# cs2mosa/Heterogeneous-MOE-for-Diffusion-models

Measured on AMD Instinct MI355X. Metric: denoise-steps/sec (fwd+bwd) on 4x32x32 latents, higher is better.
Workload: dtype bf16

## Files before the change

heterogeneous-moe-for-diffusion-models_amd/csrc/bwd6.hip:

```cpp
#include "common.h"
#include "conv_args.h"
#include "conv6_common.h"
#include "hdmoe.h"
#include "conv6_body.h"
#include "conv7_body.h"
#include "wgrad6_body.h"
#include "wgrad7_body.h"
#include "wgrad8_body.h"
#include "conv6s_body.h"

namespace {

template <int MT, int NT, int TWS, int OT>
__global__ __launch_bounds__(512) void bwd6_kernel(C6Args c, W6Args a3, W6Args a5, int G6, int ibs, int obs) {
  const int b = blockIdx.x;
  if (b < G6) { conv6_body<MT, NT>(c, b, G6); return; }
  int r = b - G6;
  const int bx = r % ibs; r /= ibs;
  const int by = r % obs;
  const int z = r / obs;
  if (z < a3.chunks) wgrad6_body<3, TWS, OT, false>(a3, bx, by, z);
  else wgrad6_body<5, TWS, OT, false>(a5, bx, by, z - a3.chunks);
}

// ... 21 lines not shown
      else if (pairs == 2) wgrad8_body3<2, 8>(a3, bx, by, z);
      else wgrad8_body3<2, 16>(a3, bx, by, z);
      return;
    }
    r -= n3;
    const int bx = r % ibs; r /= ibs;
    wgrad7_body<5>(a5, bx, r % obs, r / obs);
  } else if (OT > 0) {
    const int bx = r % ibs; r /= ibs;
    const int by = r % obs;
    const int z = r / obs;
    if (z < a3.chunks) wgrad6_body<3, TWS, OT == 0 ? 1 : OT, false>(a3, bx, by, z);
    else wgrad6_body<5, TWS, OT == 0 ? 1 : OT, false>(a5, bx, by, z - a3.chunks);
  }
}

template <int CO, int KMASK, int TWS, int OT, int EPI = 0, bool DBG = false>
void launch_bwd7(const C7Plan& cp, const W6DualPlan& wp, hipStream_t stream) {
  if constexpr (!DBG && EPI == 0 && (TWS == 5 || OT == 2)) {
    if (cp.a.stamps || cp.a.dbg) { launch_bwd7<CO, KMASK, TWS, OT, 0, true>(cp, wp, stream); return; }
  }
  static unsigned long long attr = 0;
  if (hdmoe_first_on_device(attr)) { (void)hipFuncSetAttribute((const void*)bwd7_kernel<CO, KMASK, TWS, OT, EPI, DBG>, hipFuncAttributeMaxDynamicSharedMemorySize, 160 * 1024); }
  const size_t clds = cp.lds + (EPI ? C7Lds<TWS == 4>::film_extra(CO) : 0);
  const size_t lds = clds > wp.lds ? clds : wp.lds;
  const int obs = OT == 0 ? wp.c[0].Cout / 32 : wp.obs;
  unsigned nw = (unsigned)(wp.ibs * obs * (wp.c[0].chunks + wp.c[1].chunks));
  if (OT == 0) nw = (unsigned)((wp.c[0].Cin / (32 * wp.c[0].icw)) * (wp.c[0].Cout / (32 * wp.c[0].ocw)) * wp.c[0].chunks + wp.ibs * obs * wp.c[1].chunks);
  hipLaunchKernelGGL((bwd7_kernel<CO, KMASK, TWS, OT, EPI, DBG>), dim3(cp.G + nw), dim3(512), lds, stream, cp.a, wp.c[0], wp.c[1], (int)cp.G, wp.ibs, obs);
}

template <int NT, int TWS, int OT>
__global__ __launch_bounds__(512) void bwd6s_kernel(C6SArgs c, W6Args a3, int G6, int ibs, int obs) {
  const int b = blockIdx.x;
  if (b < G6) { conv6s_body<NT>(c, b, G6); return; }
  int r = b - G6;
  const int bx = r % ibs; r /= ibs;
  wgrad6_body<3, TWS, OT, true>(a3, bx, r % obs, r / obs);
}
template <int NT, int TWS, int OT>
void launch_bwd6s(const C6SPlan& cp, const W6DualPlan& wp, hipStream_t stream) {
  static unsigned long long attr = 0;
  if (hdmoe_first_on_device(attr)) { (void)hipFuncSetAttribute((const void*)bwd6s_kernel<NT, TWS, OT>, hipFuncAttributeMaxDynamicSharedMemorySize, 160 * 1024); }
  const size_t lds = cp.lds > wp.lds ? cp.lds : wp.lds;
  const unsigned grid = cp.G + (unsigned)(wp.ibs * wp.obs * wp.c[0].chunks);
  hipLaunchKernelGGL((bwd6s_kernel<NT, TWS, OT>), dim3(grid), dim3(512), lds, stream, cp.sa, wp.c[0], (int)cp.G, wp.ibs, wp.obs);
}
// ... 72 lines not shown
  C7Plan cp7;
  if (conv7_plan(c, dtype, cp7) || cp7.kmask != 3 || (cp7.w16 != 0) != (wp.TWS == 4)) return 1;
  const bool big = wp.TWS == 5, small = wp.TWS == 4 && cp7.CO == 2 && wp.OT == 2;
  if (!big && !small) return 1;
  cp7.a.film_u = film_u; cp7.a.film_e = film_e; cp7.a.film_mask = film_mask; cp7.a.film_de = film_de;
  cp7.a.film_inv = film_p > 0.f ? 1.f / (1.f - film_p) : 1.f;
  hdmoe_count_selection(HDMOE_SEL_FILM_DGRAD);
  if (big) {
    hdmoe_count_selection(HDMOE_SEL_BWD7_32);
    if (wp.c[0].chunks) {
      hdmoe_count_selection(HDMOE_SEL_BWD7_32_WGRAD8);
      hdmoe_count_selection(wp.c[0].icw == 2 ? (wp.c[0].ocw == 2 ? HDMOE_SEL_WGRAD8_C22 : HDMOE_SEL_WGRAD8_C21)
                                             : (wp.c[0].ocw == 2 ? HDMOE_SEL_WGRAD8_C12 : HDMOE_SEL_WGRAD8_C11));
    }
    if (wp.c[1].chunks) hdmoe_count_selection(HDMOE_SEL_BWD7_32_WGRAD7);
    if (cp7.CO == 2) launch_bwd7<2, 3, 5, 0, 1>(cp7, wp, stream); else launch_bwd7<1, 3, 5, 0, 1>(cp7, wp, stream);
  } else {
    hdmoe_count_selection(HDMOE_SEL_BWD7_16_OT2);
    launch_bwd7<2, 3, 4, 2, 1>(cp7, wp, stream);
  }
  return hdmoe_launch_status();
}

}
```

heterogeneous-moe-for-diffusion-models_amd/csrc/conv7.hip:

```cpp
#include "conv_args.h"
#include "hdmoe.h"
#include "conv7_body.h"

namespace {

template <int CO, int KMASK, bool W16, bool DBG>
__global__ __launch_bounds__(512) void conv7_kernel(C7Args a) { conv7_body<CO, KMASK, W16, 0, DBG>(a, blockIdx.x, gridDim.x); }

}

constexpr int C7_MIN_IMAGES = 192;
extern "C" int hdmoe_conv7_min_images(void) { return C7_MIN_IMAGES; }

int conv7_plan(const ConvArgs& c, int dtype, C7Plan& plan) {
  if (dtype != HDMOE_BF16 || c.stride != 1 || c.ones || c.Cphys != c.Cin || c.Ipad != c.Cin || c.Cin % 32 || c.Cin > 256 || c.Cstore != c.Cout) return 1;
  if (c.Cout % 32 || c.Cout > 256) return 1;
  const bool w16 = c.H == 16;
  if (!((c.H == 32 && c.W == 32) || (c.H == 16 && c.W == 16)) || c.Ho != c.H || c.Wo != c.W || c.N < C7_MIN_IMAGES) return 1;
  int kmask = 0;
  long maxtaps = 0;
  for (int g = 0; g < c.ngroups; ++g) {
    const int k = c.kh[g];
    if (c.kw[g] != k || (k != 3 && k != 5 && k != 7) || c.pt[g] != (k - 1) / 2 || c.pl[g] != (k - 1) / 2) return 1;
    kmask |= k == 3 ? 1 : (k == 5 ? 2 : 4);
    if ((long)k * k > maxtaps) maxtaps = (long)k * k;
  }
  const long xbytes = (long)c.N * c.H * c.W * c.Cin * 2;
  const long wbytes = ((long)(c.ngroups - 1) * c.wstride + maxtaps * c.Cout * c.Cin) * 2;
  if (!conv_align_extent_ok({c.x, c.w, c.y, c.res}, {xbytes, wbytes, (long)c.N * c.H * c.W * c.Cout})) return 1;
  const long gstride = c.wstride * 2, tapstride = (long)c.Cout * c.Cin * 2, imgstride = (long)c.H * c.W * c.Cin * 2;
  if ((gstride & 7) || (c.ngroups - 1) * gstride + maxtaps * tapstride >= (1l << 31) || c.N * imgstride >= (1l << 31)) return 1;
  C7Args& a = plan.a;
  a.x = c.x; a.w = c.w; a.y = c.y; a.res = c.res; a.seg = c.seg;
  a.N = c.N; a.Cin = c.Cin; a.Cout = c.Cout; a.ngroups = c.ngroups; a.alpha = c.alpha; a.beta = c.beta;
  a.xbytes = (int)xbytes; a.wbytes = (int)wbytes;
  a.dbg = 0;
  a.film_u = nullptr; a.film_e = nullptr; a.film_mask = nullptr; a.film_de = nullptr; a.film_inv = 1.f;
  a.stamps = (unsigned long long*)hdmoe_debug_stamp_buffer();
  conv_sort_groups_desc(c.kh, a.order, c.ngroups);
  for (int i = 0; i < HDMOE_MAX_GROUPS; ++i) a.gk[i] = (int)(a.order[i] * gstride) | c.kh[a.order[i]];
  const long gcap = 256;
  const long units = w16 ? (c.N + 1) / 2 + c.ngroups : c.N;
  plan.G = (unsigned)(units < gcap ? units : gcap);
  plan.CO = c.Cout % 64 == 0 ? 2 : 1;
  a.tapstride = (int)tapstride; a.blkstride = 32 * plan.CO * c.Cin * 2;
  a.imgstride = (int)imgstride; a.rowstride = c.W * c.Cin * 2;
  plan.w16 = w16 ? 1 : 0;
  plan.lds = w16 ? C7Lds<true>::BYTES : C7Lds<false>::BYTES;
  plan.kmask = (kmask & 4) ? 7 : 3;
  return 0;
}

template <int CO, int KMASK, bool W16, bool DBG>
static void conv7_launch_t(const C7Plan& p, hipStream_t stream) {
  static unsigned long long attr = 0;
  if (hdmoe_first_on_device(attr)) { (void)hipFuncSetAttribute((const void*)conv7_kernel<CO, KMASK, W16, DBG>, hipFuncAttributeMaxDynamicSharedMemorySize, C7Lds<W16>::BYTES); }
  hipLaunchKernelGGL((conv7_kernel<CO, KMASK, W16, DBG>), dim3(p.G), dim3(512), C7Lds<W16>::BYTES, stream, p.a);
}

void conv7_launch(const C7Plan& p, hipStream_t stream) {
// ... 17 lines not shown
```

heterogeneous-moe-for-diffusion-models_amd/csrc/conv7_body.h:

```cpp
#pragma once
#include <type_traits>
#include <utility>
#include "common.h"
#include "conv6_common.h"

namespace {

struct C7Args {
  const void* x; const void* w; void* y; const void* res; const int* seg;
  int N, Cin, Cout, ngroups;
  int order[HDMOE_MAX_GROUPS];
  int gk[HDMOE_MAX_GROUPS];
  int tapstride, blkstride;
  int imgstride, rowstride;
  float alpha, beta;
  int xbytes, wbytes;
  int dbg;
  unsigned long long* stamps;
  const void* film_u;
  const float* film_e;
  const unsigned char* film_mask;
  float* film_de;
  float film_inv;
};

template <bool W16> struct C7Geo;
template <> struct C7Geo<false> {
  static constexpr int IMG = 32, MB = 4, ROWB = 35 * 64, TILE = (32 * 35 + 3) * 64, WBUF = 8192, TCO = 4, PPW = 8, HBOFF = 0;
  static constexpr int ZBYTES = 38 * 64;
};
template <> struct C7Geo<true> {
  static constexpr int IMG = 16, MB = 2, ROWB = 19 * 64, TILE = (32 * 19 + 3) * 64, WBUF = 28672, TCO = 14, PPW = 4, HBOFF = 16 * 19 * 64;
  static constexpr int ZBYTES = HBOFF + 22 * 64;
};
template <bool W16> struct C7Lds {
  using GEO = C7Geo<W16>;
  static constexpr int T0 = 2 * GEO::WBUF;
  static constexpr int ZROW = T0 + 2 * GEO::TILE;
  static constexpr int TAB = ZROW + GEO::ZBYTES;
  static constexpr int BYTES = TAB + HDMOE_MAX_GROUPS * 16;
  static constexpr int film_bytes(int co) { return 8 * (W16 ? 2 : 1) * 32 * co * 4; }
  static constexpr bool film_in_ring(int co) { return BYTES + film_bytes(co) > 160 * 1024; }
  static constexpr int film_extra(int co) { return film_in_ring(co) ? 0 : film_bytes(co); }
};

template <int KS, int CO, int TCO> struct C7Sched {
// ... 281 lines not shown
              *reinterpret_cast<bf16x8*>(Y + o) = out;
            }
          }
#pragma unroll
          for (int j = 0; j < 8; ++j) {
#pragma unroll
            for (int off = 1; off < (W16 ? 16 : 32); off <<= 1) ds[j] += __shfl_xor(ds[j], off);
          }
          if ((r & (W16 ? 15 : 31)) == 0) {
            float* dst = part + (wave * NIMG + (W16 ? (r >> 4) : 0)) * NCH + 32 * b + 16 * p + 8 * h;
            *reinterpret_cast<float4*>(dst) = make_float4(ds[0], ds[1], ds[2], ds[3]);
            *reinterpret_cast<float4*>(dst + 4) = make_float4(ds[4], ds[5], ds[6], ds[7]);
          }
        }
      asm volatile("s_waitcnt lgkmcnt(0)\n\ts_barrier" ::: "memory");
      if (tid < NIMG * NCH) {
        const int img = tid / NCH, c = tid % NCH;
        const int n = img ? cur.n2 : cur.n;
        float sum = 0.f;
#pragma unroll
        for (int w = 0; w < 8; ++w) sum += part[(w * NIMG + img) * NCH + c];
        if (n >= 0) a.film_de[(long)n * a.Cout + cobase + c] = sum;
      }
    } else if (!(dbg & 4)) {
      bf16* Y = (bf16*)a.y;
      const bf16* R = (const bf16*)a.res;
      const int nimg = W16 ? ((r >> 4) ? cur.n2 : cur.n) : cur.n;
      const bool live = !W16 || nimg >= 0;
#pragma unroll
      for (int m = 0; m < MB; ++m) {
        const long pix = W16 ? (((long)nimg * 16 + 2 * wave + m) * 16 + (r & 15)) * a.Cout
                             : (((long)nimg * 32 + 4 * wave + m) * 32 + r) * a.Cout;
#pragma unroll
        for (int b = 0; b < CO; ++b)
#pragma unroll
          for (int p = 0; p < 2; ++p) {
            float v[8];
#pragma unroll
            for (int e = 0; e < 8; ++e) v[e] = a.alpha * acc[m][b][8 * p + e];
            if (R && live) {
              const long o0 = pix + cobase + 32 * b + 16 * p + 4 * h;
              const bf16x4 r0 = *reinterpret_cast<const bf16x4*>(R + o0);
              const bf16x4 r1 = *reinterpret_cast<const bf16x4*>(R + o0 + 8);
#pragma unroll
              for (int e = 0; e < 4; ++e) { v[e] += a.beta * (float)r0[e]; v[4 + e] += a.beta * (float)r1[e]; }
            }
// ... 37 lines not shown
```

heterogeneous-moe-for-diffusion-models_amd/hdmoe_hip/ops.py:

```python
from __future__ import annotations

import ctypes
import functools
import math
from typing import Optional, Sequence, Tuple, Union

import torch

from . import bank as _bank
from ._lib import dtype_code_cast
from ._lib import BF16, _int_array, call, dtype_code, lib

Tensor = torch.Tensor

F32S = 2
ROUTE_CONV6S = 6


def _c(t: Optional[Tensor]) -> Optional[Tensor]:
    if t is None:
        return None
    return t if t.is_contiguous() else t.contiguous()


# ... 373 lines not shown
        if w6:
            return lambda: _conv_record(x, seg, N, Ho * Wo, O, I, khs, kws, "split_bf16" if split else None, wgrad_name=w6)
        return lambda: _conv_record(x, seg, N, Ho * Wo, O, I, khs, kws, wgrad_name=_kernel_label(_route(
            "hdmoe_conv_wgrad_route", 34, N, H, W, Ho, Wo, I, Cphys, O, 1, ones, G, seg is not None, khs, kws, pts, pts, _dt(x),
            x.data_ptr() % 16 == 0 and dy.data_ptr() % 16 == 0), x, wgrad=True))
    w6 = "wgrad6_kernel<split>" if split else "wgrad6_kernel"
    if (x.dtype == torch.bfloat16 or split) and not ones and Ho == H and Wo == W and Cphys == I:
        dtc = F32S if split else _dt(x)
        kib = _w6_kib(G, N, H, W, I, O, khs, kws, dtc)
        ws = _w6_workspace("arena", x.device, kib) if bank is not None and _prof_ok() else None
        if ws is not None:
            if _timed("conv_wgrad", rec(w6 + " (deferred reduce)"), "hdmoe_conv_wgrad6", x, dy, Gs, seg, G, N, H, W, I, O, khs, kws, pts, pts, ws, ws.numel() * 4,
                      dtc, 1) == 0:
                bank.defer_w6(Gs, seg, ws, G, N, H, W, I, O, dtc, khs)
                STATS["w6_defer"] += 1
                return
        ws = _w6_workspace("stream", x.device, kib)
        if ws is not None:
            if _timed("conv_wgrad", rec(w6 + " (+ reduce)"), "hdmoe_conv_wgrad6", x, dy, Gs, seg, G, N, H, W, I, O, khs, kws, pts, pts, ws, ws.numel() * 4, dtc, 0) == 0:
                return
    _timed("conv_wgrad", rec(), "hdmoe_conv_wgrad", x, dy, Gs, seg, G, N, H, W, Ho, Wo, I, Cphys, O, 1, 1 if ones else 0, khs, kws, pts, pts, _dt(x))


_ConvCall = _collections.namedtuple("_ConvCall", "G gain_val alpha beta ones training normalize split res_raw out film")


class _MPConvFn(torch.autograd.Function):

    @staticmethod
    def forward(ctx, x, res, seg, c: _ConvCall, *tensors):
        G, gain_val, alpha, beta, ones, training, normalize, split = c.G, c.gain_val, c.alpha, c.beta, c.ones, c.training, c.normalize, c.split
        weights, gains = tensors[:G], list(tensors[G:]) or None
        ctx.film = getattr(x, "_film_rec", None) if FILM_DGRAD and x.is_contiguous() else None
        if ctx.film is not None:
            ctx.film.register()
        x = _c(x)
        N, H, W, Cphys = x.shape
        O, I = int(weights[0].shape[0]), int(weights[0].shape[1])
        khs = [_kernel_hw(w)[0] for w in weights]
        kws = [_kernel_hw(w)[1] for w in weights]
        pts = [(kw - 1) // 2 for kw in kws]
        Hos = {H + (kw - 1) - kh + 1 for kh, kw in zip(khs, kws)}
        if len(Hos) != 1:
            raise ValueError("grouped conv: all groups must produce the same output size")
        if any(w.shape[0] != O or w.shape[1] != I for w in weights):
            raise ValueError("grouped conv: all groups must share (out_channels, in_channels)")
        if I != Cphys + (1 if ones else 0):
            raise RuntimeError(f"MP_Conv: input has {Cphys} channels, weight expects {I}")
        Ho, Wo = Hos.pop(), W
        Ipad = (I + 15) // 16 * 16
        Opad = (O + 15) // 16 * 16
        taps = max(a * b for a, b in zip(khs, kws))
        wstride, wdstride = taps * O * Ipad, taps * I * Opad
        wdt, planes, dtc = (torch.bfloat16, 2, F32S) if split else (x.dtype, 1, _dt(x))
        L = ctx.layer = _ConvLayer(G, N, H, W, Ho, Wo, Cphys, I, O, Ipad, Opad, khs, kws, pts, wstride, wdstride, dtc, gain_val, alpha, beta, ones,
                               normalize, split, c.res_raw, res is not None)
        ent = None
        if _bank.ACTIVE is not None and gains is None:
# ... 29 lines not shown
                    seg, G, wstride, N, H, W, Ho, Wo, I, Cphys, Ipad, O, O, 1, 1 if ones else 0, khs, kws, pts, pts, dtc)
            _timed("conv_fwd", lambda: _fwd_record(*args), "hdmoe_conv_fwd", *args)
        ctx.save_for_backward(x, seg, *tensors)
        return y

    @staticmethod
    def backward(ctx, dy):
        x, seg, *tensors = ctx.saved_tensors
        L, nig = ctx.layer, ctx.needs_input_grad
        weights, gains = tensors[:L.G], list(tensors[L.G:]) or None
        dy = _c(dy)
        need_gain = gains is not None and any(nig[4 + L.G:])
        need_w = any(nig[4:4 + L.G]) or need_gain
        fused, dx = _conv_fused_bwd(ctx, L, x, dy, seg, nig[0]) if need_w and ctx.ent is not None else (False, None)
        if nig[0] and not fused:
            dx = _conv_dgrad(L, x, dy, ctx.wd, seg)
        dres = None
        if L.has_res and nig[1]:
            if L.res_raw or L.beta == 1.0:
                dres = dy
            else:
                dres = torch.empty_like(dy)
                call("hdmoe_axpby", dres, dy, None, L.beta, 0.0, dy.numel(), _dt(dy))
        dws, dgs = _conv_wgrad(ctx, L, x, dy, seg, weights, gains, need_gain) if need_w and not fused else ([None] * L.G, [None] * len(gains or ()))
        return (dx, dres, None, None, *dws, *dgs)


def _conv_fused_bwd(ctx, L: _ConvLayer, x, dy, seg, need_dx: bool):
    rec = ctx.film
    if rec is not None:
        rec.clear()
    plan = _conv_bwd_plan(L, seg, need_dx, ctx.ones6, x.device)
    ws = plan.workspace(L, x.device) if plan is not None and plan.policy is not None else None
    if plan is None or (ws is None and plan.policy is not None):
        return False, None
    if callable(plan.mid):
        plan = plan._replace(mid=plan.mid())
    dx = torch.empty_like(x) if need_dx else None
    fused = False
    if plan.film and rec is not None and FILM_DGRAD and need_dx and rec.sole_consumer(x):
        de = torch.empty(rec.e.shape, dtype=torch.float32, device=x.device)
        fused = plan._replace(name="hdmoe_conv_bwd6_film", tail=(rec.u, rec.e, rec.mask, de, rec.p, plan.dtc),
                              label=lambda: dict(plan.label(), name="bwd7_kernel (FiLM epilogue)")).launch(ctx.bank, ctx.ent, x, dy, dx, ws)
        if fused:
            rec.offer(dx, de)
            STATS["film_dgrad"] += 1
    fused = fused or plan.launch(ctx.bank, ctx.ent, x, dy, dx, ws)
    return fused, dx if fused else None


def _conv_dgrad(L: _ConvLayer, x, dy, wd, seg) -> Tensor:
    dx = torch.empty_like(x)
    pt_d = [kh - 1 - p for kh, p in zip(L.khs, L.pts)]
    pl_d = [kw - 1 - p for kw, p in zip(L.kws, L.pts)]
    args = (dy, wd, dx, None, L.alpha, 0.0,
            seg, L.G, L.wdstride, L.N, L.Ho, L.Wo, L.H, L.W, L.O, L.O, L.Opad, L.I, L.Cphys, 1, 0, L.khs, L.kws, pt_d, pl_d, L.dtc)
    _timed("conv_fwd", lambda: _fwd_record(*args), "hdmoe_conv_fwd", *args)
    return dx


def _conv_wgrad(ctx, L: _ConvLayer, x, dy, seg, weights, gains, need_gain: bool):
    G, O, I = L.G, L.O, L.I
    geom = (seg, G, L.N, L.H, L.W, L.Ho, L.Wo, I, L.Cphys, O, L.ones, L.khs, L.kws, L.pts, L.split)
    dgs = [None] * len(gains or ())
    if ctx.ent is not None:
        _wgrad(x, dy, ctx.ent.G, *geom, bank=ctx.bank)
        ctx.bank.note_backward(ctx.ent)
        return [None] * G, dgs
    sizes = [kh * kw * O * I for kh, kw in zip(L.khs, L.kws)]
# ... 73 lines not shown
def _mp_conv(x, weights, gain=1.0, *, seg=None, res=None, alpha=1.0, beta=0.0, ones=False, training=False, normalize=True, split=False,
             res_grad_raw=False, out: Optional[Tensor] = None, film: Optional["_FilmReq"] = None) -> Tensor:
    ws = f32_params(list(weights) if isinstance(weights, (list, tuple)) else [weights])
    G = len(ws)
    if isinstance(gain, (list, tuple)):
        gts, gain_val = f32_params(list(gain)), 1.0
    elif torch.is_tensor(gain):
        gts, gain_val = f32_params([gain]) * G, 1.0
    else:
        gts, gain_val = [], float(gain)
    shape = x.shape
    grouped = seg is not None
    if x.ndim not in (2, 3, 4):
        raise ValueError("mp_conv: x must be 2-, 3- or 4-D")
    pointwise = all(w.ndim == 2 or (w.shape[2] == 1 and w.shape[3] == 1) for w in ws)
    if pointwise and not grouped and not ones:
        x4 = x.reshape(1, 1, -1, shape[-1])
    elif x.ndim == 2:
        x4 = x.reshape(shape[0], 1, 1, shape[1])
    elif x.ndim == 3:
        x4 = x.reshape(shape[0], 1, shape[1], shape[2])
    else:
        x4 = x
    if res is not None:
        res = res.reshape(x4.shape[0], x4.shape[1], x4.shape[2], -1)
    split = bool(split) and not ones and x4.dtype == torch.float32 and _split_ok(*x4.shape, ws)
    c = _ConvCall(G, gain_val, float(alpha), float(beta), bool(ones), bool(training), bool(normalize), split, bool(res_grad_raw), out, film)
    y = _MPConvFn.apply(x4, res, seg, c, *ws, *gts)
    return y.reshape(*shape[:-1], y.shape[-1])


class _MultiLinearFn(torch.autograd.Function):

    @staticmethod
    def forward(ctx, x, seg, ents, bank, c, *tensors):
        x = _f32(x)
        R, I = x.shape
        L = len(ents)
        G = len(ents[0].params)
        Os = [e.O for e in ents]
        ys = [torch.empty((R, o), dtype=torch.float32, device=x.device) for o in Os]
        call("hdmoe_mlinear_fwd", ys, x, [e.wf for e in ents], seg, Os, L, R, I, ents[0].Ipad, G, c)
        ctx.save_for_backward(x, seg)
        ctx.meta = (ents, bank, Os, G)
        return tuple(ys)

    @staticmethod
    def backward(ctx, *gs):
        x, seg = ctx.saved_tensors
        ents, bank, Os, G = ctx.meta
# ... 438 lines not shown
    def backward(ctx, g):
        return _FilmSiluFn.backward(ctx, g) + (None,)


def mp_conv_film(x: Tensor, weights, gain, emb: Tensor, p: float, training: bool, seg: Optional[Tensor] = None) -> Tensor:
    p = float(p) if training else 0.0
    C = int((weights[0] if isinstance(weights, (list, tuple)) else weights).shape[0])
    ok = (CONV_FILM and (p == 0.0 or CONV_FILM_TRAIN) and x.dtype == torch.bfloat16 and x.ndim == 4 and C % 8 == 0 and 256 % (C // 8) == 0
          and _bank.ACTIVE is not None)
    if not ok:
        return film_silu(mp_conv(x, weights, gain, seg=seg, training=training), emb, p, training)
    req = _FilmReq(_f32(emb), p, _next_seed() if p > 0.0 else 0)
    y = _mp_conv(x, weights, gain, seg=seg, training=training, film=req)
    if req.h is not None:
        return _FilmDoneFn.apply(y, req.emb, p, req.seed, req.h)
    return _FilmSiluFn.apply(y, req.emb, p, req.seed)


ONES6 = True
BLK6 = True
BLK6_SCOPE = "c32"


def unet_block_fused(h: Tensor, res: Optional[Tensor], w1s, w2s, gain1: float, gain2: float, emb: Tensor, p: float, training: bool,
                     seg: Optional[Tensor], alpha: float, beta: float, res_grad_raw: bool = False) -> Optional[Tensor]:
    w1s, w2s = list(w1s), list(w2s)
    if not (BLK6 and _bank.ACTIVE is not None and _prof_ok() and h.dtype == torch.bfloat16 and h.ndim == 4 and h.is_cuda):
        return None
    if res is not None and (res.dtype != h.dtype or not res.is_contiguous()):
        return None
    ent1 = _bank.ACTIVE.lookup(w1s, h.dtype, float(gain1), 1.0, True)
    ent2 = _bank.ACTIVE.lookup(w2s, h.dtype, float(gain2), float(alpha), True)
    if ent1 is None or ent2 is None or ent1.khs != ent1.kws or ent1.khs != ent2.khs or ent2.khs != ent2.kws:
        return None
    h = _c(h)
    N, H, W, Cin = h.shape
    C = ent1.O
    if ent1.I != Cin or ent2.I != C or ent2.O != C or (seg is None and len(w1s) != 1):
        return None
    if BLK6_SCOPE == "c32" and (C != 32 or (H == 32 and W == 32 and N >= _c7_min_images())):
        return None
    p = float(p) if training else 0.0
    e32 = _f32(emb)
    seed = _next_seed() if p > 0.0 else 0
    y = torch.empty((N, H, W, C), dtype=h.dtype, device=h.device)
    need_bwd = torch.is_grad_enabled() and (h.requires_grad or emb.requires_grad or any(w.requires_grad for w in w1s + w2s))
    u = torch.empty_like(y) if need_bwd else None
    hb = torch.empty_like(y) if need_bwd else None
    if _timed("fused", dict(name="blk6_kernel (fwd)", dtype="bfloat16", seg=seg, N=N, HW=H * W, O=C, I=Cin + C, taps=[k * k for k in ent1.khs], mult=1.0),
              "hdmoe_unet_block_fwd", h, ent1.wf, ent2.wf, u, hb, y, res, e32, seed, step_counter(h.device), p, float(alpha), float(beta), seg,
              len(w1s), ent1.wstride, ent2.wstride, N, H, W, Cin, C, ent1.khs, _dt(h)) != 0:
        if p > 0.0:
            _seed_state["ctr"] -= 1
        return None
    STATS["blk"] += 1
    if not need_bwd:
        return y
    ws1 = w1s if seg is not None else w1s[0]
    ws2 = w2s if seg is not None else w2s[0]
    uu = _mp_conv(h, ws1, gain1, seg=seg, training=training, out=u)
    hh = _FilmDoneFn.apply(uu, e32, p, seed, hb)
    return _mp_conv(hh, ws2, gain2, seg=seg, res=res, alpha=alpha, beta=beta, training=training, res_grad_raw=res_grad_raw, out=y)

# ... 42 lines not shown
        Ca, Cb = a.shape[-1], b.shape[-1]
        rows = a.numel() // Ca
        out = torch.empty((*a.shape[:-1], Ca + Cb), dtype=a.dtype, device=a.device)
        call("hdmoe_cat2_fwd", out, a, b, wa, wb, Ca, Cb, rows, _dt(a))
        ctx.meta = (wa, wb, a.shape, b.shape)
        return out

    @staticmethod
    def backward(ctx, g):
        wa, wb, sa, sb = ctx.meta
        g = _c(g)
        da = torch.empty(sa, dtype=g.dtype, device=g.device)
        db = torch.empty(sb, dtype=g.dtype, device=g.device)
        call("hdmoe_cat2_bwd", da, db, g, wa, wb, sa[-1], sb[-1], da.numel() // sa[-1], _dt(g))
        return da, db, None, None


def mp_cat(a: Tensor, b: Tensor, t: float = 0.5) -> Tensor:
    na, nb = a.shape[-1], b.shape[-1]
    c = math.sqrt((na + nb) / ((1.0 - t) ** 2 + t ** 2))
    return _Cat2Fn.apply(a, b, c * (1.0 - t) / math.sqrt(na), c * t / math.sqrt(nb))


class _SiluBranchFn(torch.autograd.Function):

    @staticmethod
    def forward(ctx, x, gx_scale):
        ctx.set_materialize_grads(False)
        x = _c(x)
        h = torch.empty_like(x)
        call("hdmoe_mp_silu_fwd", h, x, x.numel(), _dt(x))
        ctx.save_for_backward(x)
        ctx.sx = float(gx_scale)
        return x.view(x.shape), h

    @staticmethod
    def backward(ctx, gx, gh):
        (x,) = ctx.saved_tensors
        if gh is None:
            if gx is None or ctx.sx == 1.0:
                return gx, None
            dx = torch.empty_like(x)
            call("hdmoe_axpby", dx, _c(gx), None, ctx.sx, 0.0, dx.numel(), _dt(dx))
            return dx, None
        gh = _c(gh)
        dx = torch.empty_like(x)
        if gx is None:
            call("hdmoe_mp_silu_bwd", dx, gh, x, x.numel(), _dt(x))
        else:
            call("hdmoe_mp_silu_bwd_add", dx, gh, x, _c(gx), ctx.sx, x.numel(), _dt(x))
        return dx, None


class _CatSiluFn(torch.autograd.Function):

    @staticmethod
    def forward(ctx, a, b, wa, wb):
        ctx.set_materialize_grads(False)
        a = _c(a); b = _c(b)
        Ca, Cb = a.shape[-1], b.shape[-1]
        out = torch.empty((*a.shape[:-1], Ca + Cb), dtype=a.dtype, device=a.device)
        h = torch.empty_like(out)
        call("hdmoe_cat2_silu_fwd", out, h, a, b, wa, wb, Ca, Cb, a.numel() // Ca, _dt(a))
        ctx.save_for_backward(out)
        ctx.meta = (wa, wb, a.shape, b.shape)
        return out, h

    @staticmethod
    def backward(ctx, gcat, gh):
        (out,) = ctx.saved_tensors
        wa, wb, sa, sb = ctx.meta
        da = torch.empty(sa, dtype=out.dtype, device=out.device)
        db = torch.empty(sb, dtype=out.dtype, device=out.device)
        if gh is None:
            if gcat is None:
                return None, None, None, None
            call("hdmoe_cat2_bwd", da, db, _c(gcat), wa, wb, sa[-1], sb[-1], da.numel() // sa[-1], _dt(out))
        else:
            call("hdmoe_cat2_silu_bwd", da, db, None if gcat is None else _c(gcat), _c(gh), out, wa, wb, sa[-1], sb[-1], da.numel() // sa[-1], _dt(out))
        return da, db, None, None


def _vec_ok(*ts) -> bool:
    return all(t.shape[-1] % (8 if t.dtype == torch.bfloat16 else 4) == 0 and t.dtype in (torch.bfloat16, torch.float32) for t in ts)


def silu_branch(x: Tensor, gx_scale: float = 1.0):
    if _vec_ok(x) and x.numel() % 8 == 0:
        return _SiluBranchFn.apply(x, float(gx_scale))
    x, xh = fanout(x, 2)
    if gx_scale != 1.0:
        x = affine_grad(x, gx_scale)
    return x, mp_silu(xh)

# ... 1587 lines not shown
```

heterogeneous-moe-for-diffusion-models_amd/models/model_components.py:

```python
from __future__ import annotations

from typing import List, Optional, Sequence

import torch
import torch.nn as nn

import models.model_internals as m
from hdmoe_hip import ops

Tensor = torch.Tensor


class Scaling_router(nn.Module):

    def __init__(self, emb_dim: Optional[int] = 3, num_experts: Optional[int] = 2, dropout: Optional[float] = 0.2):
        super().__init__()
        self.soft_route = nn.Sequential(
            m.MP_Conv(in_channels=emb_dim, out_channels=emb_dim * 2, kernel=()),
            nn.GroupNorm(1, emb_dim * 2),
            nn.ReLU(),
            m.MP_Conv(in_channels=emb_dim * 2, out_channels=emb_dim * 4, kernel=()),
            nn.GroupNorm(1, emb_dim * 4),
            nn.ReLU(),
            nn.Dropout(dropout),
# ... 92 lines not shown

    def conv(name, inp, gain=1.0, **kw):
        return ops.mp_conv(inp, [getattr(b, name).weights for b in blocks], gain, seg=seg, training=tr, **kw)

    emb = film if film is not None else ops.affine(conv("emb_layer", embedding, b0.emb_gain), 1.0, 1.0)
    x = ops.resample(x, b0.resample)
    t = b0.residual_balance
    n = ((1.0 - t) ** 2 + t ** 2) ** 0.5
    beta = (1.0 - t) / n
    raw = False
    if b0.type == "enc":
        if b0.conv_skip is not None:
            x = conv("conv_skip", x)
        x, h = ops.pixel_norm_silu(x, gx_scale=beta)
        raw = True
    elif silu_x is not None:
        h = silu_x
    else:
        skip_next = b0.conv_skip is not None
        x, h = ops.silu_branch(x, gx_scale=1.0 if skip_next else beta)
        raw = not skip_next
    w1, w2 = [b.conv_res1.weights for b in blocks], [b.conv_res2.weights for b in blocks]
    if b0.type == "dec" and b0.conv_skip is not None:
        x = conv("conv_skip", x, alpha=beta)
        rbeta, raw = 1.0, False
    else:
        rbeta = beta
    yb = ops.unet_block_fused(h, x, w1, w2, b0.conv_gain1, b0.conv_gain2, emb, b0.dropout, tr, seg, alpha=t / n, beta=rbeta, res_grad_raw=raw)
    if yb is not None:
        return yb
    y = ops.mp_conv_film(h, w1, b0.conv_gain1, emb, b0.dropout, tr, seg=seg)
    return conv("conv_res2", y, b0.conv_gain2, res=x, alpha=t / n, beta=rbeta, res_grad_raw=raw)


class Unet_block(nn.Module):

    def __init__(self, in_channels: int, out_channels: int, kernel: tuple, emb_size: int, resample: Optional[str] = "keep",
                 Type: Optional[str] = "enc", residual_balance: Optional[float] = 0.5, Dropout: Optional[float] = 0.2,
                 emb_gain: Optional[float] = 1.0, conv_gain: Optional[float] = 1.0):
        super().__init__()
        self.in_channels = in_channels
        self.out_channels = out_channels
        self.emb_size = emb_size
        self.residual_balance = residual_balance
        self.type = Type
        self.resample = resample
        self.kernel = kernel
        self.dropout = Dropout
# ... 343 lines not shown
```

include/hdmoe.h:

```cpp
#ifndef HDMOE_H
#define HDMOE_H
#ifdef __cplusplus
extern "C" {
#endif

#ifndef HDMOE_OK
#define HDMOE_OK 0
#define HDMOE_EINVAL (-1)
#define HDMOE_EDTYPE (-2)
#define HDMOE_ELAUNCH (-3)
#define HDMOE_F32 0
#define HDMOE_BF16 1
#define HDMOE_F16 3
#define HDMOE_F32S 2
#define HDMOE_MAX_GROUPS 8
#endif

typedef void* hdmoe_stream_t;
#ifdef __HIPCC__
#define HS hipStream_t
#else
#define HS hdmoe_stream_t
#endif

// ... 4 lines not shown
                    int normalize, int mutate, int flip, int dtype, HS stream);
int hdmoe_wprep_bwd(const float* const* w_raw, const float* const* gain_ptr, float gain_val, const float* const* G,
                    float* const* dw, float* const* dgain, const int* kh, const int* kw, int ngroups, int O, int I,
                    int normalize, HS stream);
int hdmoe_conv_fwd(const void* x, const void* w, void* y, const void* res, float alpha, float beta, const int* seg,
                   int ngroups, long wstride, int N, int H, int W, int Ho, int Wo, int Cin, int Cphys, int Ipad, int Cout,
                   int Cstore, int stride, int ones, const int* kh, const int* kw, const int* pt, const int* pl, int dtype,
                   HS stream);
int hdmoe_conv_wgrad(const void* x, const void* dy, float* const* G, const int* seg, int ngroups, int N, int H, int W,
                     int Ho, int Wo, int Cin, int Cphys, int Cout, int stride, int ones, const int* kh, const int* kw,
                     const int* pt, const int* pl, int dtype, HS stream);

int hdmoe_conv_wgrad6_ws_kib(int ngroups, int N, int H, int W, int Cin, int Cout, const int* kh, const int* kw, int dtype);
int hdmoe_conv_wgrad6(const void* x, const void* dy, float* const* G, const int* seg, int ngroups, int N, int H, int W, int Cin,
                      int Cout, const int* kh, const int* kw, const int* pt, const int* pl, void* ws, long ws_bytes, int dtype,
                      int defer, HS stream);
int hdmoe_conv_bwd6(const void* x, const void* dy, const void* wd, void* dx, float* const* G, const int* seg, int ngroups,
                    long wd_stride, int N, int H, int W, int Cin, int Cout, const int* kh, const int* kw, const int* pt,
                    const int* pl, float alpha, void* ws, long ws_bytes, int dtype, HS stream);
int hdmoe_conv_bwd6_film(const void* x, const void* dy, const void* wd, void* dx, float* const* G, const int* seg, int ngroups,
                         long wd_stride, int N, int H, int W, int Cin, int Cout, const int* kh, const int* kw, const int* pt,
                         const int* pl, float alpha, void* ws, long ws_bytes, const void* film_u, const float* film_e,
                         const unsigned char* film_mask, float* film_de, float film_p, int dtype, HS stream);
int hdmoe_pw_bwd(const void* x, const void* dy, const void* wd, void* dx, float* const* G, const int* seg, int ngroups,
                 long wd_stride, int N, long HW, int Cin, int Cout, float alpha, int dtype, HS stream);
int hdmoe_conv_bwd6s(const void* x, const void* dy, const void* wd, void* dx, float* const* G, const int* seg, int ngroups,
                     long wd_stride, long wd_plane, int N, int H, int W, int Cin, int Cout, const int* kh, const int* kw,
                     const int* pt, const int* pl, float alpha, void* ws, long ws_bytes, const float* in_scale, const float* in_shift,
                     int in_relu, int hi_only, HS stream);
int hdmoe_conv_fwd_split_gn(const void* x, const void* w, void* y, const float* in_scale, const float* in_shift, int in_relu,
                            float* stats_ws, long wstride, long wplane, int N, int H, int W, int Cin, int Cout, float alpha, HS stream);
int hdmoe_conv_fwd_film(const void* x, const void* w, void* y, void* h, const float* e, unsigned long long seed,
                        const unsigned long long* seed_dev, float p, float alpha, const int* seg, int ngroups, long wstride, int N, int H, int W,
                        int Cin, int Cout, const int* kh, const int* kw, const int* pt, const int* pl, int dtype, HS stream);
int hdmoe_conv_split_stats_slots(int H, int W, int Cout);
int hdmoe_gn1_finalize(float* scale, float* shift, float* mean, float* rstd, const float* ws, const float* gamma, const float* beta,
                       int N, int slots, int C, long count, float eps, HS stream);
int hdmoe_gn1_relu_mean(float* out, const float* y, const float* scale, const float* shift, int N, long S, int C, HS stream);
int hdmoe_gn1_finalize_relu_mean(float* out, float* scale, float* shift, float* mean, float* rstd, const float* y, const float* ws,
                                 const float* gamma, const float* beta, int N, int slots, long S, int C, float eps, HS stream);
int hdmoe_gn1_finalize_relu_mean_pq(float* out, float* scale, float* shift, float* mean, float* rstd, float* pcnt, float* qsum, const float* y,
                                    const float* ws, const float* gamma, const float* beta, int N, int slots, long S, int C, float eps, HS stream);
int hdmoe_conv_wgrad6_reduce_batch(float* const* G, const int* const* seg, float* const* ws, const int* dims, int n, HS stream);

int hdmoe_conv6_debug_stamps(void* buf);

// ... 2 lines not shown
  HDMOE_SEL_CONV7_16 = 1,
  HDMOE_SEL_CONV6 = 2,
  HDMOE_SEL_CONV6S = 3,
  HDMOE_SEL_BWD7_32 = 4,
  HDMOE_SEL_BWD7_32_WGRAD8 = 5,
  HDMOE_SEL_BWD7_32_WGRAD7 = 6,
  HDMOE_SEL_BWD7_16_OT1 = 7,
  HDMOE_SEL_BWD7_16_OT2 = 8,
  HDMOE_SEL_BWD6 = 9,
  HDMOE_SEL_BWD6S = 10,
  HDMOE_SEL_WGRAD6_DIRECT = 11,
  HDMOE_SEL_WGRAD6_DEFER = 12,
  HDMOE_SEL_BLK6 = 13,
  HDMOE_SEL_WGRAD8_C11 = 14,
  HDMOE_SEL_WGRAD8_C12 = 15,
  HDMOE_SEL_WGRAD8_C21 = 16,
  HDMOE_SEL_WGRAD8_C22 = 17,
  HDMOE_SEL_PW_BWD = 18,
  HDMOE_SEL_RELAYOUT_TILED = 19,
  HDMOE_SEL_COMBINE_FWD_VEC = 20,
  HDMOE_SEL_COMBINE_BWD_VEC = 21,
  HDMOE_SEL_FILM_DGRAD = 22,
  HDMOE_SEL_ROW_WINDOW = 23,
  HDMOE_SEL_COUNT = 24
};
int hdmoe_kernel_selections(long long* counts, int n, int reset);

enum {
  HDMOE_ROUTE_CONV_FWD = 0,
  HDMOE_ROUTE_CONV_FWD2 = 1,
  HDMOE_ROUTE_CONV_FWD3 = 2,
  HDMOE_ROUTE_CONV_FWD5 = 3,
  HDMOE_ROUTE_CONV_CONV7 = 4,
  HDMOE_ROUTE_CONV_CONV6 = 5,
  HDMOE_ROUTE_CONV_CONV6S = 6,
  HDMOE_ROUTE_CONV_KGEMM = 7,
  HDMOE_ROUTE_CONV_GLIN = 8,
  HDMOE_ROUTE_CONV_NONE = 9,
  HDMOE_ROUTE_CONV_ROWLIN = 10,
  HDMOE_ROUTE_WGRAD_V2 = 0,
  HDMOE_ROUTE_WGRAD_V1 = 1,
  HDMOE_ROUTE_WGRAD_SWG = 2,
  HDMOE_ROUTE_WGRAD_TOWG = 3,
  HDMOE_ROUTE_WGRAD_LWG = 4
};
int hdmoe_conv_fwd_route(int* route, int N, int H, int W, int Ho, int Wo, int Cin, int Cphys, int Ipad, int Cout, int Cstore, int stride, int ones,
                         int ngroups, int has_seg, int has_res, long wstride, const int* kh, const int* kw, const int* pt, const int* pl,
// ... 287 lines not shown
```

Baseline: 86.77.

## Fuse SiLU/cat-SiLU activation backward into conv7 dgrad epilogue

Adds an EPI==2 epilogue to the conv7 dgrad kernel that applies the mp-SiLU gradient, optionally adds the incoming skip gradient, and splits output channels for the concatenated case. A Python-side _ActRec protocol hands the activation input and the pending source gradient to the conv backward, so the separate SiLU/cat backward kernels and their extra reads and writes of dx are skipped. The decoder skip block is also rerouted to the unfused film path outside the fused-block scope so this epilogue can apply there. It brings in bookkeeping across autograd nodes and a runtime error if an activation output feeds more than one consumer.

```diff
diff --git a/heterogeneous-moe-for-diffusion-models_amd/csrc/bwd6.hip b/heterogeneous-moe-for-diffusion-models_amd/csrc/bwd6.hip
--- a/heterogeneous-moe-for-diffusion-models_amd/csrc/bwd6.hip
+++ b/heterogeneous-moe-for-diffusion-models_amd/csrc/bwd6.hip
@@ -67,7 +67,7 @@
   }
   static unsigned long long attr = 0;
   if (hdmoe_first_on_device(attr)) { (void)hipFuncSetAttribute((const void*)bwd7_kernel<CO, KMASK, TWS, OT, EPI, DBG>, hipFuncAttributeMaxDynamicSharedMemorySize, 160 * 1024); }
-  const size_t clds = cp.lds + (EPI ? C7Lds<TWS == 4>::film_extra(CO) : 0);
+  const size_t clds = cp.lds + (EPI == 1 ? C7Lds<TWS == 4>::film_extra(CO) : 0);
   const size_t lds = clds > wp.lds ? clds : wp.lds;
   const int obs = OT == 0 ? wp.c[0].Cout / 32 : wp.obs;
   unsigned nw = (unsigned)(wp.ibs * obs * (wp.c[0].chunks + wp.c[1].chunks));
@@ -186,4 +186,38 @@
   return hdmoe_launch_status();
 }
 
-}
+int hdmoe_conv_bwd6_act(const void* x, const void* dy, const void* wd, void* dx, float* const* G, const int* seg, int ngroups, long wd_stride,
+                        int N, int H, int W, int Cin, int Cout, const int* kh, const int* kw, const int* pt, const int* pl, float alpha,
+                        void* ws, long ws_bytes, const void* act_x, const void* act_g, float act_sx, void* dx2, int act_ca, float act_wa,
+                        float act_wb, int dtype, hipStream_t stream) {
+  if (dtype != HDMOE_BF16 || !dx || !wd || ngroups < 1 || ngroups > HDMOE_MAX_GROUPS || Cout % 16) return 1;
+  if (!act_x || ((uintptr_t)act_x & 15) || ((uintptr_t)act_g & 15) || ((uintptr_t)dx2 & 15)) return 1;
+  if (act_ca < 0 || act_ca >= Cin || (act_ca > 0) != (dx2 != nullptr)) return HDMOE_EINVAL;
+  if (act_ca % 32) return 1;
+  W6DualPlan wp;
+  if (wgrad6_plan_dual(x, dy, G, seg, ngroups, N, H, W, Cin, Cout, kh, kw, pt, pl, ws, ws_bytes, dtype, wp)) return 1;
+  const ConvArgs c = conv_dgrad_args(dy, wd, dx, seg, ngroups, wd_stride, N, H, W, Cin, Cout, kh, kw, pt, pl, alpha);
+  C7Plan cp7;
+  if (conv7_plan(c, dtype, cp7) || cp7.kmask != 3 || (cp7.w16 != 0) != (wp.TWS == 4)) return 1;
+  const bool big = wp.TWS == 5, small = wp.TWS == 4 && cp7.CO == 2 && wp.OT == 2;
+  if (!big && !small) return 1;
+  cp7.a.act_x = act_x; cp7.a.act_g = act_g; cp7.a.act_sx = act_sx; cp7.a.y2 = dx2; cp7.a.act_ca = act_ca;
+  cp7.a.act_wa = act_ca > 0 ? act_wa : 1.f; cp7.a.act_wb = act_ca > 0 ? act_wb : 1.f;
+  hdmoe_count_selection(HDMOE_SEL_ACT_DGRAD);
+  if (big) {
+    hdmoe_count_selection(HDMOE_SEL_BWD7_32);
+    if (wp.c[0].chunks) {
+      hdmoe_count_selection(HDMOE_SEL_BWD7_32_WGRAD8);
+      hdmoe_count_selection(wp.c[0].icw == 2 ? (wp.c[0].ocw == 2 ? HDMOE_SEL_WGRAD8_C22 : HDMOE_SEL_WGRAD8_C21)
+                                             : (wp.c[0].ocw == 2 ? HDMOE_SEL_WGRAD8_C12 : HDMOE_SEL_WGRAD8_C11));
+    }
+    if (wp.c[1].chunks) hdmoe_count_selection(HDMOE_SEL_BWD7_32_WGRAD7);
+    if (cp7.CO == 2) launch_bwd7<2, 3, 5, 0, 2>(cp7, wp, stream); else launch_bwd7<1, 3, 5, 0, 2>(cp7, wp, stream);
+  } else {
+    hdmoe_count_selection(HDMOE_SEL_BWD7_16_OT2);
+    launch_bwd7<2, 3, 4, 2, 2>(cp7, wp, stream);
+  }
+  return hdmoe_launch_status();
+}
+
+}
diff --git a/heterogeneous-moe-for-diffusion-models_amd/csrc/conv7.hip b/heterogeneous-moe-for-diffusion-models_amd/csrc/conv7.hip
--- a/heterogeneous-moe-for-diffusion-models_amd/csrc/conv7.hip
+++ b/heterogeneous-moe-for-diffusion-models_amd/csrc/conv7.hip
@@ -36,6 +36,7 @@
   a.xbytes = (int)xbytes; a.wbytes = (int)wbytes;
   a.dbg = 0;
   a.film_u = nullptr; a.film_e = nullptr; a.film_mask = nullptr; a.film_de = nullptr; a.film_inv = 1.f;
+  a.act_x = nullptr; a.act_g = nullptr; a.y2 = nullptr; a.act_sx = 1.f; a.act_wa = 1.f; a.act_wb = 1.f; a.act_ca = 0;
   a.stamps = (unsigned long long*)hdmoe_debug_stamp_buffer();
   conv_sort_groups_desc(c.kh, a.order, c.ngroups);
   for (int i = 0; i < HDMOE_MAX_GROUPS; ++i) a.gk[i] = (int)(a.order[i] * gstride) | c.kh[a.order[i]];
diff --git a/heterogeneous-moe-for-diffusion-models_amd/csrc/conv7_body.h b/heterogeneous-moe-for-diffusion-models_amd/csrc/conv7_body.h
--- a/heterogeneous-moe-for-diffusion-models_amd/csrc/conv7_body.h
+++ b/heterogeneous-moe-for-diffusion-models_amd/csrc/conv7_body.h
@@ -22,6 +22,11 @@
   const unsigned char* film_mask;
   float* film_de;
   float film_inv;
+  const void* act_x;
+  const void* act_g;
+  void* y2;
+  float act_sx, act_wa, act_wb;
+  int act_ca;
 };
 
 template <bool W16> struct C7Geo;
@@ -349,6 +354,71 @@
         for (int w = 0; w < 8; ++w) sum += part[(w * NIMG + img) * NCH + c];
         if (n >= 0) a.film_de[(long)n * a.Cout + cobase + c] = sum;
       }
+    } else if constexpr (EPI == 2) {
+      const bf16* X = (const bf16*)a.act_x;
+      const bf16* GX = (const bf16*)a.act_g;
+      const int nimg = W16 ? ((r >> 4) ? cur.n2 : cur.n) : cur.n;
+      const bool live = !W16 || nimg >= 0;
+      const int ca = a.act_ca;
+      C6Words pk[CO][2][MB];
+#pragma unroll
+      for (int b = 0; b < CO; ++b)
+#pragma unroll
+        for (int p = 0; p < 2; ++p)
+#pragma unroll
+          for (int m = 0; m < MB; ++m) {
+            float v[8];
+#pragma unroll
+            for (int e = 0; e < 8; ++e) v[e] = a.alpha * acc[m][b][8 * p + e];
+            pk[b][p][m] = c6_pack_bf16(v);
+          }
+      const long pix0 = W16 ? ((long)nimg * 16 + 2 * wave) * 16 + (r & 15) : ((long)nimg * 32 + 4 * wave) * 32 + r;
+#pragma unroll
+      for (int b = 0; b < CO; ++b) {
+        bf16x8 xx[2][MB], gg[2][MB];
+        __builtin_amdgcn_sched_barrier(0);
+        if (live) {
+#pragma unroll
+          for (int p = 0; p < 2; ++p)
+#pragma unroll
+            for (int m = 0; m < MB; ++m)
+              xx[p][m] = *reinterpret_cast<const bf16x8*>(X + (pix0 + m * IMG) * a.Cout + cobase + 32 * b + 16 * p + 8 * h);
+          if (GX) {
+#pragma unroll
+            for (int p = 0; p < 2; ++p)
+#pragma unroll
+              for (int m = 0; m < MB; ++m)
+                gg[p][m] = *reinterpret_cast<const bf16x8*>(GX + (pix0 + m * IMG) * a.Cout + cobase + 32 * b + 16 * p + 8 * h);
+          }
+        }
+        __builtin_amdgcn_sched_barrier(0);
+#pragma unroll
+        for (int p = 0; p < 2; ++p) {
+          const int c0 = cobase + 32 * b + 16 * p + 8 * h;
+          const bool second = ca > 0 && c0 >= ca;
+          bf16* D = (bf16*)(second ? a.y2 : a.y);
+          const int dC = ca > 0 ? (second ? a.Cout - ca : ca) : a.Cout, dc = second ? c0 - ca : c0;
+          const float wgt = second ? a.act_wb : a.act_wa;
+#pragma unroll
+          for (int m = 0; m < MB; ++m) {
+            if (live) {
+              bf16x8 out;
+#pragma unroll
+              for (int j = 0; j < 8; ++j) {
+                const unsigned wj = pk[b][p][m].w[j >> 1];
+                const float g = __uint_as_float((j & 1) ? (wj & 0xFFFF0000u) : (wj << 16));
+                const float sg = mp_silu_grad_f((float)xx[p][m][j]);
+                float f;
+                if (ca > 0) f = __builtin_fmaf(sg, g, GX ? (float)gg[p][m][j] : 0.f) * wgt;
+                else if (GX) f = __builtin_fmaf(a.act_sx, (float)gg[p][m][j], g * sg);
+                else f = g * sg;
+                out[j] = (bf16)f;
+              }
+              *reinterpret_cast<bf16x8*>(D + (pix0 + m * IMG) * dC + dc) = out;
+            }
+          }
+        }
+      }
     } else if (!(dbg & 4)) {
       bf16* Y = (bf16*)a.y;
       const bf16* R = (const bf16*)a.res;
diff --git a/heterogeneous-moe-for-diffusion-models_amd/hdmoe_hip/ops.py b/heterogeneous-moe-for-diffusion-models_amd/hdmoe_hip/ops.py
--- a/heterogeneous-moe-for-diffusion-models_amd/hdmoe_hip/ops.py
+++ b/heterogeneous-moe-for-diffusion-models_amd/hdmoe_hip/ops.py
@@ -419,7 +419,7 @@
     _timed("conv_wgrad", rec(), "hdmoe_conv_wgrad", x, dy, Gs, seg, G, N, H, W, Ho, Wo, I, Cphys, O, 1, 1 if ones else 0, khs, kws, pts, pts, _dt(x))
 
 
-_ConvCall = _collections.namedtuple("_ConvCall", "G gain_val alpha beta ones training normalize split res_raw out film")
+_ConvCall = _collections.namedtuple("_ConvCall", "G gain_val alpha beta ones training normalize split res_raw out film act_src")
 
 
 class _MPConvFn(torch.autograd.Function):
@@ -431,6 +431,13 @@
         ctx.film = getattr(x, "_film_rec", None) if FILM_DGRAD and x.is_contiguous() else None
         if ctx.film is not None:
             ctx.film.register()
+        ctx.act = getattr(x, "_act_rec", None) if ACT_DGRAD and x.is_contiguous() else None
+        if ctx.act is not None:
+            ctx.act.register()
+        ctx.act_src = c.act_src if ACT_DGRAD else None
+        for rec in ctx.act_src or ():
+            if rec is not None:
+                rec.register_source()
         x = _c(x)
         N, H, W, Cphys = x.shape
         O, I = int(weights[0].shape[0]), int(weights[0].shape[1])
@@ -506,14 +513,19 @@
             else:
                 dres = torch.empty_like(dy)
                 call("hdmoe_axpby", dres, dy, None, L.beta, 0.0, dy.numel(), _dt(dy))
+        for rec, g in zip(ctx.act_src or (), (dx, dres)):
+            if rec is not None:
+                rec.deliver(g)
         dws, dgs = _conv_wgrad(ctx, L, x, dy, seg, weights, gains, need_gain) if need_w and not fused else ([None] * L.G, [None] * len(gains or ()))
         return (dx, dres, None, None, *dws, *dgs)
 
 
 def _conv_fused_bwd(ctx, L: _ConvLayer, x, dy, seg, need_dx: bool):
-    rec = ctx.film
+    rec, act = ctx.film, ctx.act
     if rec is not None:
         rec.clear()
+    if act is not None:
+        act.clear()
     plan = _conv_bwd_plan(L, seg, need_dx, ctx.ones6, x.device)
     ws = plan.workspace(L, x.device) if plan is not None and plan.policy is not None else None
     if plan is None or (ws is None and plan.policy is not None):
@@ -529,6 +541,21 @@
         if fused:
             rec.offer(dx, de)
             STATS["film_dgrad"] += 1
+    if not fused and plan.film and act is not None and ACT_DGRAD and need_dx and act.sole_consumer(x) and act.ready():
+        got = act.take()
+        if act.cat is None:
+            parts, tail = (dx,), (act.x, got, act.sx, None, 0, 1.0, 1.0, plan.dtc)
+        else:
+            wa, wb, Ca = act.cat
+            parts = tuple(torch.empty((*x.shape[:-1], C), dtype=x.dtype, device=x.device) for C in (Ca, x.shape[-1] - Ca))
+            tail = (act.x, got, 1.0, parts[1], Ca, wa, wb, plan.dtc)
+        fused = plan._replace(name="hdmoe_conv_bwd6_act", tail=tail,
+                              label=lambda: dict(plan.label(), name="bwd7_kernel (activation epilogue)")).launch(ctx.bank, ctx.ent, x, dy, parts[0], ws)
+        if fused:
+            if act.cat is not None:
+                dx = torch.empty((), dtype=x.dtype, device=x.device).expand(x.shape)
+            act.offer(dx, got, parts)
+            STATS["act_dgrad"] += 1
     fused = fused or plan.launch(ctx.bank, ctx.ent, x, dy, dx, ws)
     return fused, dx if fused else None
 
@@ -648,10 +675,13 @@
         x4 = x.reshape(shape[0], 1, shape[1], shape[2])
     else:
         x4 = x
+    res0 = res
     if res is not None:
         res = res.reshape(x4.shape[0], x4.shape[1], x4.shape[2], -1)
     split = bool(split) and not ones and x4.dtype == torch.float32 and _split_ok(*x4.shape, ws)
-    c = _ConvCall(G, gain_val, float(alpha), float(beta), bool(ones), bool(training), bool(normalize), split, bool(res_grad_raw), out, film)
+    act_src = (getattr(x, "_act_src", None), getattr(res0, "_act_src", None))
+    c = _ConvCall(G, gain_val, float(alpha), float(beta), bool(ones), bool(training), bool(normalize), split, bool(res_grad_raw), out, film,
+                  act_src if any(r is not None for r in act_src) else None)
     y = _MPConvFn.apply(x4, res, seg, c, *ws, *gts)
     return y.reshape(*shape[:-1], y.shape[-1])
 
@@ -1136,6 +1166,10 @@
 BLK6_SCOPE = "c32"
 
 
+def unet_block_fused_in_scope(N: int, H: int, W: int, C: int) -> bool:
+    return BLK6 and not (BLK6_SCOPE == "c32" and (C != 32 or (H == 32 and W == 32 and N >= _c7_min_images())))
+
+
 def unet_block_fused(h: Tensor, res: Optional[Tensor], w1s, w2s, gain1: float, gain2: float, emb: Tensor, p: float, training: bool,
                      seg: Optional[Tensor], alpha: float, beta: float, res_grad_raw: bool = False) -> Optional[Tensor]:
     w1s, w2s = list(w1s), list(w2s)
@@ -1152,7 +1186,7 @@
     C = ent1.O
     if ent1.I != Cin or ent2.I != C or ent2.O != C or (seg is None and len(w1s) != 1):
         return None
-    if BLK6_SCOPE == "c32" and (C != 32 or (H == 32 and W == 32 and N >= _c7_min_images())):
+    if not unet_block_fused_in_scope(N, H, W, C):
         return None
     p = float(p) if training else 0.0
     e32 = _f32(emb)
@@ -1241,6 +1275,55 @@
     return _Cat2Fn.apply(a, b, c * (1.0 - t) / math.sqrt(na), c * t / math.sqrt(nb))
 
 
+class _ActRec:
+    __slots__ = ("x", "sx", "cat", "taken", "src_taken", "_got", "_offer")
+
+    def __init__(self, x, sx, cat=None):
+        self.x, self.sx, self.cat = x, sx, cat
+        self.taken = self.src_taken = 0
+        self._got = self._offer = None
+
+    def register(self) -> None:
+        self.taken += 1
+
+    def register_source(self) -> None:
+        self.src_taken += 1
+
+    def sole_consumer(self, h: Tensor) -> bool:
+        return self.taken == 1 and self.x.shape == h.shape and self.x.dtype == h.dtype
+
+    def deliver(self, g: Optional[Tensor]) -> None:
+        ok = g is not None and self.src_taken == 1 and g.dtype == self.x.dtype and g.numel() == self.x.numel() and g.is_contiguous()
+        self._got = g if ok else None
+
+    def ready(self) -> bool:
+        return self.src_taken == 0 or self._got is not None
+
+    def take(self) -> Optional[Tensor]:
+        got, self._got = self._got, None
+        return got
+
+    def clear(self) -> None:
+        self._offer = None
+
+    def offer(self, gh: Tensor, got: Optional[Tensor], parts: tuple) -> None:
+        self._offer = (gh, got, parts)
+
+    def claim(self, gx: Optional[Tensor], gh: Optional[Tensor]):
+        offer, self._offer, self._got = self._offer, None, None
+        if offer is None:
+            return None
+        tok, got, parts = offer
+        same = lambda a, b: (a is None and b is None) or (a is not None and b is not None and a.data_ptr() == b.data_ptr() and a.numel() == b.numel())
+        if gh is None or gh.data_ptr() != tok.data_ptr() or gh.shape != tok.shape or not same(gx, got):
+            raise RuntimeError("silu_branch / mp_cat_silu: an output fed a second consumer beside the conv layers that fused its backward "
+                               "(set ops.ACT_DGRAD = False)")
+        return parts
+
+
+ACT_DGRAD = True
+
+
 class _SiluBranchFn(torch.autograd.Function):
 
     @staticmethod
@@ -1251,11 +1334,18 @@
         call("hdmoe_mp_silu_fwd", h, x, x.numel(), _dt(x))
         ctx.save_for_backward(x)
         ctx.sx = float(gx_scale)
-        return x.view(x.shape), h
+        xv = x.view(x.shape)
+        ctx.rec = None
+        if x.dtype == torch.bfloat16 and x.ndim == 4:
+            ctx.rec = h._act_rec = xv._act_src = _ActRec(x, ctx.sx)
+        return xv, h
 
     @staticmethod
     def backward(ctx, gx, gh):
         (x,) = ctx.saved_tensors
+        done = ctx.rec.claim(gx, gh) if ctx.rec is not None else None
+        if done is not None:
+            return done[0], None
         if gh is None:
             if gx is None or ctx.sx == 1.0:
                 return gx, None
@@ -1283,12 +1373,18 @@
         call("hdmoe_cat2_silu_fwd", out, h, a, b, wa, wb, Ca, Cb, a.numel() // Ca, _dt(a))
         ctx.save_for_backward(out)
         ctx.meta = (wa, wb, a.shape, b.shape)
+        ctx.rec = None
+        if out.dtype == torch.bfloat16 and out.ndim == 4:
+            ctx.rec = h._act_rec = out._act_src = _ActRec(out, 1.0, (float(wa), float(wb), Ca))
         return out, h
 
     @staticmethod
     def backward(ctx, gcat, gh):
         (out,) = ctx.saved_tensors
         wa, wb, sa, sb = ctx.meta
+        done = ctx.rec.claim(gcat, gh) if ctx.rec is not None else None
+        if done is not None:
+            return done[0], done[1], None, None
         da = torch.empty(sa, dtype=out.dtype, device=out.device)
         db = torch.empty(sb, dtype=out.dtype, device=out.device)
         if gh is None:
diff --git a/heterogeneous-moe-for-diffusion-models_amd/models/model_components.py b/heterogeneous-moe-for-diffusion-models_amd/models/model_components.py
--- a/heterogeneous-moe-for-diffusion-models_amd/models/model_components.py
+++ b/heterogeneous-moe-for-diffusion-models_amd/models/model_components.py
@@ -138,8 +138,12 @@
         raw = not skip_next
     w1, w2 = [b.conv_res1.weights for b in blocks], [b.conv_res2.weights for b in blocks]
     if b0.type == "dec" and b0.conv_skip is not None:
-        x = conv("conv_skip", x, alpha=beta)
         rbeta, raw = 1.0, False
+        skip = lambda: conv("conv_skip", x, alpha=beta)
+        if h.ndim == 4 and not ops.unet_block_fused_in_scope(h.shape[0], h.shape[1], h.shape[2], w1[0].shape[0]):
+            y = ops.mp_conv_film(h, w1, b0.conv_gain1, emb, b0.dropout, tr, seg=seg)
+            return conv("conv_res2", y, b0.conv_gain2, res=skip(), alpha=t / n, beta=rbeta, res_grad_raw=raw)
+        x = skip()
     else:
         rbeta = beta
     yb = ops.unet_block_fused(h, x, w1, w2, b0.conv_gain1, b0.conv_gain2, emb, b0.dropout, tr, seg, alpha=t / n, beta=rbeta, res_grad_raw=raw)
diff --git a/include/hdmoe.h b/include/hdmoe.h
--- a/include/hdmoe.h
+++ b/include/hdmoe.h
@@ -50,6 +50,10 @@
                          long wd_stride, int N, int H, int W, int Cin, int Cout, const int* kh, const int* kw, const int* pt,
                          const int* pl, float alpha, void* ws, long ws_bytes, const void* film_u, const float* film_e,
                          const unsigned char* film_mask, float* film_de, float film_p, int dtype, HS stream);
+int hdmoe_conv_bwd6_act(const void* x, const void* dy, const void* wd, void* dx, float* const* G, const int* seg, int ngroups,
+                        long wd_stride, int N, int H, int W, int Cin, int Cout, const int* kh, const int* kw, const int* pt,
+                        const int* pl, float alpha, void* ws, long ws_bytes, const void* act_x, const void* act_g, float act_sx,
+                        void* dx2, int act_ca, float act_wa, float act_wb, int dtype, HS stream);
 int hdmoe_pw_bwd(const void* x, const void* dy, const void* wd, void* dx, float* const* G, const int* seg, int ngroups,
                  long wd_stride, int N, long HW, int Cin, int Cout, float alpha, int dtype, HS stream);
 int hdmoe_conv_bwd6s(const void* x, const void* dy, const void* wd, void* dx, float* const* G, const int* seg, int ngroups,
@@ -98,7 +102,8 @@
   HDMOE_SEL_COMBINE_BWD_VEC = 21,
   HDMOE_SEL_FILM_DGRAD = 22,
   HDMOE_SEL_ROW_WINDOW = 23,
-  HDMOE_SEL_COUNT = 24
+  HDMOE_SEL_ACT_DGRAD = 24,
+  HDMOE_SEL_COUNT = 25
 };
 int hdmoe_kernel_selections(long long* counts, int n, int reset);
 
```

After: 87.49, median of 6. Within noise of the previous version (+0.8%).
